# SorF520/D2R

Measured on AMD Instinct MI355X. Metric: samples/sec fwd+bwd, higher is better.
Workload: dtype fp16

## Files before the change

d2r_amd/csrc/attention_impl.inc:

```
typedef H16<E>::v8 E8;
typedef H16<E>::v4 E4;

namespace {

struct MhaArgs {
  const E *q, *k, *v, *res, *dO;
  E *o, *dq, *dk, *dv;
  const float* mask;
  float* lse;
  float* dsum;
  uint32_t drop_thresh;
  float drop_scale;
  uint64_t drop_seed;
  int lkp;
  int64_t ldq, sqb, ldk, skb, ldv, svb, ldo, sob, ldr, srb, ldg, sgb, lddq, sdqb, lddk, sdkb, lddv, sdvb;
  int B, H, Lq, Lk;
  float scale;
};

constexpr int LDW = 72;

template <int DH, int TOTAL, int NTHREADS>
struct RowStage {
  static constexpr int CHUNKS = TOTAL * 8, IT = (CHUNKS + NTHREADS - 1) / NTHREADS;
// ... 9 lines not shown
    }
  }
  __device__ __forceinline__ void store(E* dst, int tid) const {
#pragma unroll
    for (int it = 0; it < IT; ++it) {
      const int c = tid + it * NTHREADS, row = c >> 3, col = (c & 7) * 8;
      if (CHUNKS % NTHREADS == 0 || c < CHUNKS) st_pack<E, 8>(dst + row * LDW + col, v[it]);
    }
  }
};

template <int DH, int TOTAL, int NTHREADS>
__device__ __forceinline__ void fill_rows(E* dst, const E* src, int64_t ld, int valid, int tid) {
  RowStage<DH, TOTAL, NTHREADS> r;
  r.load(src, ld, valid, tid);
  r.store(dst, tid);
}

template <int DH, int TOTAL, int NTHREADS>
__device__ __forceinline__ void fill_rows2(E* d0, const E* s0, int64_t ld0, int v0, E* d1, const E* s1, int64_t ld1, int v1, int tid) {
  RowStage<DH, TOTAL, NTHREADS> r0, r1;
  r0.load(s0, ld0, v0, tid);
  r1.load(s1, ld1, v1, tid);
  r0.store(d0, tid);
  r1.store(d1, tid);
}

__device__ __forceinline__ E8 lds_frag(const E* p) { return *reinterpret_cast<const E8*>(p); }

__device__ __forceinline__ E8 lds_frag_tr(const E* base, int k0, int c0, int tq, int tp) {
  const E* p0 = base + (k0 + tq) * LDW + c0 + tp * 4;
  const E4 lo = H16<E>::tr_read(p0);
  const E4 hi = H16<E>::tr_read(p0 + 16 * LDW);
  return E8{lo[0], lo[1], lo[2], lo[3], hi[0], hi[1], hi[2], hi[3]};
}

__device__ __forceinline__ E8 pack_frag(const f32x4& a, const f32x4& b) {
  return E8{(E)a[0], (E)a[1], (E)a[2], (E)a[3], (E)b[0], (E)b[1], (E)b[2], (E)b[3]};
}

__device__ __forceinline__ float group4_max(float v) {
  v = fmaxf(v, __shfl_xor(v, 16, 64));
  return fmaxf(v, __shfl_xor(v, 32, 64));
}
__device__ __forceinline__ float group4_sum(float v) {
  v += __shfl_xor(v, 16, 64);
  return v + __shfl_xor(v, 32, 64);
}

__device__ __forceinline__ float drop_mult(const MhaArgs& a, uint64_t row_base, int key) {
  return d2r_rand24(a.drop_seed, row_base + (uint64_t)key) >= a.drop_thresh ? a.drop_scale : 0.f;
}

template <int DH, int NK32>
__global__ __launch_bounds__(512) void mha_fwd_kernel(MhaArgs a) {
  constexpr int LKP = NK32 * 32, NKT = NK32 * 2, NDT = DH / 16, NW = 8;
  __shared__ __attribute__((aligned(16))) E Ks[LKP * LDW];
  __shared__ __attribute__((aligned(16))) E Vs[LKP * LDW];
  __shared__ __attribute__((aligned(16))) float Ms[LKP];
  const int tid = threadIdx.x, lane = tid & 63, wave = tid >> 6;
  const int fr = lane & 15, fq = lane >> 4, tq = fr >> 2, tp = fr & 3;
  const int b = blockIdx.x / a.H, h = blockIdx.x % a.H;
  const int nqt = (a.Lq + 15) / 16;
  E8 qn[2];
  auto loadq = [&](int qt) {
    const int qrow = min(qt * 16 + fr, a.Lq - 1);
    const E* Qg = a.q + b * a.sqb + h * DH + (int64_t)qrow * a.ldq;
#pragma unroll
    for (int kk = 0; kk < 2; ++kk) {
      const int col = kk * 32 + fq * 8;
      if (col < DH) {
        qn[kk] = *reinterpret_cast<const E8*>(Qg + col);
      } else {
#pragma unroll
        for (int j = 0; j < 8; ++j) qn[kk][j] = (E)0.f;
      }
    }
  };
  if (wave < nqt) loadq(wave);
  fill_rows2<DH, LKP, 512>(Ks, a.k + b * a.skb + h * DH, a.ldk, a.Lk, Vs, a.v + b * a.svb + h * DH, a.ldv, a.Lk, tid);
  for (int key = tid; key < LKP; key += 512)
    Ms[key] = key < a.Lk ? (a.mask ? a.mask[(int64_t)b * a.Lk + key] : 0.f) : -INFINITY;
  __syncthreads();
  for (int qt = wave; qt < nqt; qt += NW) {
    asm volatile("" ::: "memory");
    const int qrow = qt * 16 + fr;
    const bool qok = qrow < a.Lq;
    E8 qf[2] = {qn[0], qn[1]};
    if (qt + NW < nqt) loadq(qt + NW);
    f32x4 s[NKT];
    float mx = -INFINITY;
#pragma unroll
    for (int t = 0; t < NKT; ++t) {
      f32x4 acc = {0.f, 0.f, 0.f, 0.f};
#pragma unroll
      for (int kk = 0; kk < 2; ++kk)
        acc = H16<E>::mfma32(lds_frag(&Ks[(t * 16 + fr) * LDW + kk * 32 + fq * 8]), qf[kk], acc);
      const f32x4 m4 = *reinterpret_cast<const f32x4*>(&Ms[t * 16 + fq * 4]);
#pragma unroll
      for (int r = 0; r < 4; ++r) {
        acc[r] = acc[r] * a.scale + m4[r];
        mx = fmaxf(mx, acc[r]);
      }
      s[t] = acc;
    }
    mx = group4_max(mx);
    float sum = 0.f;
#pragma unroll
    for (int t = 0; t < NKT; ++t)
#pragma unroll
      for (int r = 0; r < 4; ++r) {
        s[t][r] = __expf(s[t][r] - mx);
        sum += s[t][r];
      }
    sum = group4_sum(sum);
    const float inv = 1.f / sum;
    if (fq == 0 && qok) a.lse[((int64_t)b * a.H + h) * a.Lq + qrow] = mx + logf(sum);
    if (a.drop_thresh) {
      const uint64_t rb = (((uint64_t)b * a.H + h) * a.Lq + (qok ? qrow : 0)) * a.lkp;
#pragma unroll
      for (int t = 0; t < NKT; ++t)
#pragma unroll
        for (int r = 0; r < 4; ++r) s[t][r] *= drop_mult(a, rb, t * 16 + fq * 4 + r);
    }
    f32x4 o[NDT];
#pragma unroll
    for (int dt = 0; dt < NDT; ++dt) o[dt] = f32x4{0.f, 0.f, 0.f, 0.f};
#pragma unroll
    for (int u = 0; u < NK32; ++u) {
      const E8 pf = pack_frag(s[2 * u] * inv, s[2 * u + 1] * inv);
#pragma unroll
      for (int dt = 0; dt < NDT; ++dt)
        o[dt] = H16<E>::mfma32(lds_frag_tr(Vs, u * 32 + fq * 4, dt * 16, tq, tp), pf, o[dt]);
    }
    if (!qok) continue;
    E* Og = a.o + b * a.sob + h * DH + (int64_t)qrow * a.ldo;
    const E* Rg = a.res ? a.res + b * a.srb + h * DH + (int64_t)qrow * a.ldr : nullptr;
#pragma unroll
    for (int dt = 0; dt < NDT; ++dt) {
      const int c = dt * 16 + fq * 4;
      Pack<E, 4> out;
      if (Rg) {
        const Pack<E, 4> rv = ld_pack<E, 4>(Rg + c);
#pragma unroll
        for (int r = 0; r < 4; ++r) out.v[r] = (E)(o[dt][r] + (float)rv.v[r]);
      } else {
#pragma unroll
        for (int r = 0; r < 4; ++r) out.v[r] = (E)o[dt][r];
      }
      st_pack<E, 4>(Og + c, out);
    }
  }
}

template <int DH>
__device__ __forceinline__ E8 global_frag(const E* slice, int64_t ld, int row, int valid, int kk, int fq) {
  const int col = kk * 32 + fq * 8;
  const bool ok = row < valid && col < DH;
  E8 v = *reinterpret_cast<const E8*>(slice + (ok ? (int64_t)row * ld + col : 0));
#pragma unroll
  for (int j = 0; j < 8; ++j) v[j] = ok ? v[j] : (E)0.f;
  return v;
}

template <int DH, int NK32>
__global__ __launch_bounds__(512) void mha_bwd_kernel(MhaArgs a) {
  constexpr int LP = NK32 * 32, NT16 = NK32 * 2, NDT = DH / 16, NW = 8;
  __shared__ __attribute__((aligned(16))) E Xs[LP * LDW];
  __shared__ __attribute__((aligned(16))) E Ys[LP * LDW];
  __shared__ __attribute__((aligned(16))) float Ms[LP];
  __shared__ __attribute__((aligned(16))) float Ls[LP];
  __shared__ __attribute__((aligned(16))) float Ds[LP];
  E* const Ks = Xs;
  E* const Vs = Ys;
  E* const Qs = Xs;
  E* const Gs = Ys;
  const int tid = threadIdx.x, lane = tid & 63, wave = tid >> 6;
  const int fr = lane & 15, fq = lane >> 4, tq = fr >> 2, tp = fr & 3;
  const int b = blockIdx.x / a.H, h = blockIdx.x % a.H;
  const E* Qg = a.q + b * a.sqb + h * DH;
  const E* Kg = a.k + b * a.skb + h * DH;
  const E* Vg = a.v + b * a.svb + h * DH;
  const E* Gg = a.dO + b * a.sgb + h * DH;
  const int nqt = (a.Lq + 15) / 16, nkt = (a.Lk + 15) / 16;
  E8 fx[2], fy[2];
  auto fetch = [&](const E* X, int64_t ldx, const E* Y, int64_t ldy, int row0, int valid) {
#pragma unroll
    for (int kk = 0; kk < 2; ++kk) {
      fx[kk] = global_frag<DH>(X, ldx, row0 + fr, valid, kk, fq);
      fy[kk] = global_frag<DH>(Y, ldy, row0 + fr, valid, kk, fq);
    }
  };
  if (wave < nqt) fetch(Qg, a.ldq, Gg, a.ldg, wave * 16, a.Lq);
  fill_rows2<DH, LP, 512>(Ks, Kg, a.ldk, a.Lk, Vs, Vg, a.ldv, a.Lk, tid);
  for (int i = tid; i < LP; i += 512) {
    Ms[i] = i < a.Lk ? (a.mask ? a.mask[(int64_t)b * a.Lk + i] : 0.f) : -INFINITY;
    Ls[i] = i < a.Lq ? a.lse[((int64_t)b * a.H + h) * a.Lq + i] : INFINITY;
    Ds[i] = 0.f;
  }
  __syncthreads();

  for (int qt = wave; qt < nqt; qt += NW) {
    const int q0 = qt * 16;
    if (qt != wave) fetch(Qg, a.ldq, Gg, a.ldg, q0, a.Lq);
    E8 (&qf)[2] = fx, (&gf)[2] = fy;
    const float lse = Ls[q0 + fr];
    const uint64_t rbA = (((uint64_t)b * a.H + h) * a.Lq + min(q0 + fr, a.Lq - 1)) * a.lkp;
    auto tile = [&](int t, f32x4& pv, f32x4& dpv) {
      f32x4 sa = {0.f, 0.f, 0.f, 0.f}, da = {0.f, 0.f, 0.f, 0.f};
#pragma unroll
      for (int kk = 0; kk < 2; ++kk) {
        sa = H16<E>::mfma32(lds_frag(&Ks[(t * 16 + fr) * LDW + kk * 32 + fq * 8]), qf[kk], sa);
        da = H16<E>::mfma32(lds_frag(&Vs[(t * 16 + fr) * LDW + kk * 32 + fq * 8]), gf[kk], da);
      }
      const f32x4 m4 = *reinterpret_cast<const f32x4*>(&Ms[t * 16 + fq * 4]);
#pragma unroll
      for (int r = 0; r < 4; ++r) sa[r] = __expf(sa[r] * a.scale + m4[r] - lse);
      if (a.drop_thresh) {
#pragma unroll
        for (int r = 0; r < 4; ++r) da[r] *= drop_mult(a, rbA, t * 16 + fq * 4 + r);
      }
      pv = sa;
      dpv = da;
    };
    float dsum = 0.f;
#pragma unroll 2
    for (int t = 0; t < NT16; ++t) {
      f32x4 pv, dpv;
      tile(t, pv, dpv);
#pragma unroll
      for (int r = 0; r < 4; ++r) dsum += pv[r] * dpv[r];
    }
    dsum = group4_sum(dsum);
    if (fq == 0) Ds[q0 + fr] = dsum;
    f32x4 dq[NDT];
#pragma unroll
    for (int dt = 0; dt < NDT; ++dt) dq[dt] = f32x4{0.f, 0.f, 0.f, 0.f};
#pragma unroll 1
    for (int u = 0; u < NK32; ++u) {
      f32x4 p0, p1, d0, d1;
      tile(2 * u, p0, d0);
      tile(2 * u + 1, p1, d1);
#pragma unroll
      for (int r = 0; r < 4; ++r) {
        d0[r] = p0[r] * (d0[r] - dsum) * a.scale;
        d1[r] = p1[r] * (d1[r] - dsum) * a.scale;
      }
      const E8 dsf = pack_frag(d0, d1);
#pragma unroll
      for (int dt = 0; dt < NDT; ++dt)
        dq[dt] = H16<E>::mfma32(lds_frag_tr(Ks, u * 32 + fq * 4, dt * 16, tq, tp), dsf, dq[dt]);
    }
    if (q0 + fr < a.Lq) {
      E* dQg = a.dq + b * a.sdqb + h * DH + (int64_t)(q0 + fr) * a.lddq;
#pragma unroll
      for (int dt = 0; dt < NDT; ++dt) {
        Pack<E, 4> out;
#pragma unroll
        for (int r = 0; r < 4; ++r) out.v[r] = (E)dq[dt][r];
        st_pack<E, 4>(dQg + dt * 16 + fq * 4, out);
      }
    }
  }
  if (wave < nkt) fetch(Kg, a.ldk, Vg, a.ldv, wave * 16, a.Lk);
  __syncthreads();
  fill_rows2<DH, LP, 512>(Qs, Qg, a.ldq, a.Lq, Gs, Gg, a.ldg, a.Lq, tid);
  __syncthreads();

  for (int kt = wave; kt < nkt; kt += NW) {
    const int k0 = kt * 16;
    if (kt != wave) fetch(Kg, a.ldk, Vg, a.ldv, k0, a.Lk);
    E8 (&kf)[2] = fx, (&vf)[2] = fy;
    const float mk = Ms[k0 + fr];
    f32x4 dk[NDT], dv[NDT];
#pragma unroll
    for (int dt = 0; dt < NDT; ++dt) {
      dk[dt] = f32x4{0.f, 0.f, 0.f, 0.f};
      dv[dt] = f32x4{0.f, 0.f, 0.f, 0.f};
    }
#pragma unroll 1
    for (int u = 0; u < NK32; ++u) {
      f32x4 pt[2], dst[2];
#pragma unroll
      for (int half = 0; half < 2; ++half) {
        const int r0 = (u * 2 + half) * 16;
        f32x4 sa = {0.f, 0.f, 0.f, 0.f}, da = {0.f, 0.f, 0.f, 0.f};
#pragma unroll
        for (int kk = 0; kk < 2; ++kk) {
          sa = H16<E>::mfma32(lds_frag(&Qs[(r0 + fr) * LDW + kk * 32 + fq * 8]), kf[kk], sa);
          da = H16<E>::mfma32(lds_frag(&Gs[(r0 + fr) * LDW + kk * 32 + fq * 8]), vf[kk], da);
        }
        const f32x4 l4 = *reinterpret_cast<const f32x4*>(&Ls[r0 + fq * 4]);
        const f32x4 d4 = *reinterpret_cast<const f32x4*>(&Ds[r0 + fq * 4]);
#pragma unroll
        for (int r = 0; r < 4; ++r) {
          const float pv = __expf(sa[r] * a.scale + mk - l4[r]);
          float mlt = 1.f;
          if (a.drop_thresh)
            mlt = drop_mult(a, (((uint64_t)b * a.H + h) * a.Lq + min(r0 + fq * 4 + r, a.Lq - 1)) * a.lkp, min(k0 + fr, a.Lk - 1));
          pt[half][r] = pv * mlt;
          dst[half][r] = pv * (da[r] * mlt - d4[r]) * a.scale;
        }
      }
      const E8 pf = pack_frag(pt[0], pt[1]), dsf = pack_frag(dst[0], dst[1]);
#pragma unroll
      for (int dt = 0; dt < NDT; ++dt) {
        dv[dt] = H16<E>::mfma32(lds_frag_tr(Gs, u * 32 + fq * 4, dt * 16, tq, tp), pf, dv[dt]);
        dk[dt] = H16<E>::mfma32(lds_frag_tr(Qs, u * 32 + fq * 4, dt * 16, tq, tp), dsf, dk[dt]);
      }
    }
    if (k0 + fr < a.Lk) {
      E* dKg = a.dk + b * a.sdkb + h * DH + (int64_t)(k0 + fr) * a.lddk;
      E* dVg = a.dv + b * a.sdvb + h * DH + (int64_t)(k0 + fr) * a.lddv;
#pragma unroll
      for (int dt = 0; dt < NDT; ++dt) {
        Pack<E, 4> ok, ov;
#pragma unroll
        for (int r = 0; r < 4; ++r) {
          ok.v[r] = (E)dk[dt][r];
          ov.v[r] = (E)dv[dt][r];
        }
        st_pack<E, 4>(dKg + dt * 16 + fq * 4, ok);
        st_pack<E, 4>(dVg + dt * 16 + fq * 4, ov);
      }
// ... 247 lines not shown
    for (int u = 0; u < NK32; ++u) {
      f32x4 pt[2], dst[2];
#pragma unroll
      for (int half = 0; half < 2; ++half) {
        const int r0 = (u * 2 + half) * 16;
        f32x4 sa = {0.f, 0.f, 0.f, 0.f}, da = {0.f, 0.f, 0.f, 0.f};
#pragma unroll
        for (int kk = 0; kk < 2; ++kk) {
          sa = H16<E>::mfma32(lds_frag(&Qs[(r0 + fr) * LDW + kk * 32 + fq * 8]), kf[kk], sa);
          da = H16<E>::mfma32(lds_frag(&Gs[(r0 + fr) * LDW + kk * 32 + fq * 8]), vf[kk], da);
        }
        const f32x4 l4 = *reinterpret_cast<const f32x4*>(&Ls[r0 + fq * 4]);
        const f32x4 d4 = *reinterpret_cast<const f32x4*>(&Ds[r0 + fq * 4]);
#pragma unroll
        for (int r = 0; r < 4; ++r) {
          const float pv = __expf(sa[r] * a.scale + mk - l4[r]);
          float mlt = 1.f;
          if (a.drop_thresh)
            mlt = drop_mult(a, (((uint64_t)b * a.H + h) * a.Lq + min(q0 + r0 + fq * 4 + r, a.Lq - 1)) * a.lkp, kok ? krow : 0);
          pt[half][r] = pv * mlt;
          dst[half][r] = pv * (da[r] * mlt - d4[r]) * a.scale;
        }
      }
      const E8 pf = pack_frag(pt[0], pt[1]), dsf = pack_frag(dst[0], dst[1]);
#pragma unroll
      for (int dt = 0; dt < NDT; ++dt) {
        dv[dt] = H16<E>::mfma32(lds_frag_tr(Gs, u * 32 + fq * 4, dt * 16, tq, tp), pf, dv[dt]);
        dk[dt] = H16<E>::mfma32(lds_frag_tr(Qs, u * 32 + fq * 4, dt * 16, tq, tp), dsf, dk[dt]);
      }
    }
  }
  if (!kok) return;
  E* dKg = a.dk + b * a.sdkb + h * DH + (int64_t)krow * a.lddk;
  E* dVg = a.dv + b * a.sdvb + h * DH + (int64_t)krow * a.lddv;
#pragma unroll
  for (int dt = 0; dt < NDT; ++dt) {
    Pack<E, 4> ok, ov;
#pragma unroll
    for (int r = 0; r < 4; ++r) {
      ok.v[r] = (E)dk[dt][r];
      ov.v[r] = (E)dv[dt][r];
    }
    st_pack<E, 4>(dKg + dt * 16 + fq * 4, ok);
    st_pack<E, 4>(dVg + dt * 16 + fq * 4, ov);
  }
}

bool aligned_slice(const void* p, int64_t ld, int64_t sb, int dh) {
  return p && (reinterpret_cast<uintptr_t>(p) & 15u) == 0 && ld % 8 == 0 && sb % 8 == 0 && (dh * 2) % 16 == 0;
}

template <int DH>
void launch_fwd(const MhaArgs& a, int nk32, hipStream_t st) {
  const dim3 grid(a.B * a.H), block(512);
  switch (nk32) {
#define D2R_CASE(N) case N: hipLaunchKernelGGL((mha_fwd_kernel<DH, N>), grid, block, 0, st, a); break;
    D2R_CASE(1) D2R_CASE(2) D2R_CASE(3) D2R_CASE(4) D2R_CASE(5) D2R_CASE(6) D2R_CASE(7) D2R_CASE(8)
#undef D2R_CASE
  }
  d2r_attn_note(D2R_AV_MHA_FWD + DH * 100 + nk32);
}
template <int DH>
void launch_bwd(const MhaArgs& a, int nk32, hipStream_t st) {
  const dim3 grid(a.B * a.H), block(512);
  switch (nk32) {
#define D2R_CASE(N) case N: hipLaunchKernelGGL((mha_bwd_kernel<DH, N>), grid, block, 0, st, a); break;
    D2R_CASE(1) D2R_CASE(2) D2R_CASE(3) D2R_CASE(4) D2R_CASE(5) D2R_CASE(6) D2R_CASE(7) D2R_CASE(8)
#undef D2R_CASE
  }
  d2r_attn_note(D2R_AV_MHA_BWD + DH * 100 + nk32);
}

}

int mha_fwd_run(int dtype, const void* q, int64_t ldq, int64_t sqb, const void* k, int64_t ldk, int64_t skb,
                           const void* v, int64_t ldv, int64_t svb, void* o, int64_t ldo, int64_t sob,
                           const void* residual, int64_t ldr, int64_t srb, const float* mask, float* lse, int B, int H,
                           int Lq, int Lk, int head_dim, float scale, float p_drop, uint64_t seed, void* stream) {
  D2R_REQUIRE(p_drop >= 0.f && p_drop < 1.f, "d2r_mha_fwd: dropout probability must be in [0, 1)");
  D2R_REQUIRE(d2r_mha_supported(dtype, Lq, Lk, head_dim), "d2r_mha_fwd: unsupported (16-bit dtype, head_dim 64|48, L <= 1024 only)");
  D2R_REQUIRE(B >= 1 && H >= 1 && lse, "d2r_mha_fwd: bad arguments");
  D2R_REQUIRE(aligned_slice(q, ldq, sqb, head_dim) && aligned_slice(k, ldk, skb, head_dim) && aligned_slice(v, ldv, svb, head_dim) &&
                  aligned_slice(o, ldo, sob, head_dim) && (!residual || aligned_slice(residual, ldr, srb, head_dim)),
              "d2r_mha_fwd: pointers must be 16-byte aligned, strides multiples of 8 elements");
  MhaArgs a = {};
  a.q = (const E*)q, a.k = (const E*)k, a.v = (const E*)v, a.res = (const E*)residual, a.o = (E*)o;
  a.mask = mask, a.lse = lse;
  a.ldq = ldq, a.sqb = sqb, a.ldk = ldk, a.skb = skb, a.ldv = ldv, a.svb = svb, a.ldo = ldo, a.sob = sob, a.ldr = ldr, a.srb = srb;
  a.B = B, a.H = H, a.Lq = Lq, a.Lk = Lk, a.scale = scale;
  a.drop_thresh = p_drop > 0.f ? d2r_drop_threshold(p_drop) : 0u, a.drop_scale = 1.f / (1.f - p_drop), a.drop_seed = seed, a.lkp = (Lk + 7) / 8 * 8;
  if (Lq > 256 || Lk > 256) {
    const dim3 grid(d2r_cdiv(Lq, LB), B * H);
    if (head_dim == 64) hipLaunchKernelGGL(mha_long_fwd_kernel<64>, grid, dim3(512), 0, (hipStream_t)stream, a);
    else hipLaunchKernelGGL(mha_long_fwd_kernel<48>, grid, dim3(512), 0, (hipStream_t)stream, a);
    d2r_attn_note(D2R_AV_MHA_LONG_FWD + head_dim * 100);
    return d2r_check_launch("d2r_mha_fwd(long)");
  }
  const int nk32 = d2r_cdiv(Lk, 32);
  if (head_dim == 64) launch_fwd<64>(a, nk32, (hipStream_t)stream);
  else launch_fwd<48>(a, nk32, (hipStream_t)stream);
  return d2r_check_launch("d2r_mha_fwd");
}

int mha_bwd_run(int dtype, const void* q, int64_t ldq, int64_t sqb, const void* k, int64_t ldk, int64_t skb,
                           const void* v, int64_t ldv, int64_t svb, const void* dO, int64_t ldg, int64_t sgb,
                           const float* mask, const float* lse, float* dsum, void* dq, int64_t lddq, int64_t sdqb, void* dk,
                           int64_t lddk, int64_t sdkb, void* dv, int64_t lddv, int64_t sdvb, int B, int H, int Lq, int Lk,
                           int head_dim, float scale, float p_drop, uint64_t seed, void* stream) {
  D2R_REQUIRE(p_drop >= 0.f && p_drop < 1.f, "d2r_mha_bwd: dropout probability must be in [0, 1)");
  D2R_REQUIRE(d2r_mha_supported(dtype, Lq, Lk, head_dim), "d2r_mha_bwd: unsupported (16-bit dtype, head_dim 64|48, L <= 1024 only)");
  D2R_REQUIRE((Lq <= 256 && Lk <= 256) || dsum, "d2r_mha_bwd: sequences above 256 tokens need the dsum scratch ([B, H, Lq] fp32)");
  D2R_REQUIRE(B >= 1 && H >= 1 && lse, "d2r_mha_bwd: bad arguments");
  D2R_REQUIRE(aligned_slice(q, ldq, sqb, head_dim) && aligned_slice(k, ldk, skb, head_dim) && aligned_slice(v, ldv, svb, head_dim) &&
                  aligned_slice(dO, ldg, sgb, head_dim) && aligned_slice(dq, lddq, sdqb, head_dim) &&
                  aligned_slice(dk, lddk, sdkb, head_dim) && aligned_slice(dv, lddv, sdvb, head_dim),
              "d2r_mha_bwd: pointers must be 16-byte aligned, strides multiples of 8 elements");
  MhaArgs a = {};
// ... 307 lines not shown
```

d2r_amd/csrc/rowops.hip:

```cpp
#include "common.h"

template <typename TX, typename TY, int MAXPL>
__global__ __launch_bounds__(256) void softmax_fwd_kernel(const TX* __restrict__ X, TY* __restrict__ Y, int64_t ld,
                                                          int64_t rows, int cols, float scale,
                                                          const float* __restrict__ mask, int64_t rows_per_mask) {
  const int lane = threadIdx.x & 63;
  const int64_t row = (int64_t)blockIdx.x * 4 + (threadIdx.x >> 6);
  if (row >= rows) return;
  const TX* x = X + row * ld;
  const float* mk = mask ? mask + (row / rows_per_mask) * cols : nullptr;
  float v[MAXPL];
  float mx = -INFINITY;
#pragma unroll
  for (int i = 0; i < MAXPL; ++i) {
    const int c = lane + i * 64;
    if (c < cols) {
      float t = scale * to_f<TX>(x[c]);
      if (mk) t += mk[c];
      v[i] = t;
      mx = fmaxf(mx, t);
    } else {
      v[i] = -INFINITY;
    }
  }
// ... 206 lines not shown
#pragma unroll
  for (int i = 0; i < MAXP; ++i) {
    const int pk = lane + i * 64, pc = pk < npk ? pk : 0;
    px[i] = ld_pack<T, VEC>(x + pc * VEC);
#pragma unroll
    for (int j = 0; j < VEC; j += 4) {
      const float4 g4 = *reinterpret_cast<const float4*>(gamma + pc * VEC + j);
      const float4 b4 = *reinterpret_cast<const float4*>(beta + pc * VEC + j);
      gm[i][j] = g4.x, gm[i][j + 1] = g4.y, gm[i][j + 2] = g4.z, gm[i][j + 3] = g4.w;
      bt[i][j] = b4.x, bt[i][j + 1] = b4.y, bt[i][j + 2] = b4.z, bt[i][j + 3] = b4.w;
    }
  }
  __builtin_amdgcn_sched_barrier(0);
#pragma unroll
  for (int i = 0; i < MAXP; ++i) {
    const float mk = lane + i * 64 < npk ? 1.f : 0.f;
#pragma unroll
    for (int j = 0; j < VEC; ++j) {
      v[i][j] = to_f<T>(px[i].v[j]);
      s += v[i][j] * mk;
    }
  }
  const float mu = wave_sum(s) / D;
  float q = 0.f;
#pragma unroll
  for (int i = 0; i < MAXP; ++i) {
    const int pk = lane + i * 64;
    if (pk < npk) {
#pragma unroll
      for (int j = 0; j < VEC; ++j) {
        const float d = v[i][j] - mu;
        q += d * d;
      }
    }
  }
  const float rs = rsqrtf(wave_sum(q) / D + eps);
  if (lane == 0) {
    mean[row] = mu;
    rstd[row] = rs;
  }
  T* y = Y + row * D;
#pragma unroll
  for (int i = 0; i < MAXP; ++i) {
    const int pk = lane + i * 64;
    if (pk < npk) {
      Pack<T, VEC> o;
#pragma unroll
      for (int j = 0; j < VEC; ++j) o.v[j] = from_f<T>((v[i][j] - mu) * rs * gm[i][j] + bt[i][j]);
      st_pack<T, VEC>(y + pk * VEC, o);
    }
  }
}

template <typename T, int MAXP>
__global__ __launch_bounds__(256) void layernorm_bwd_kernel(const T* __restrict__ dY, const T* __restrict__ X,
                                                            const float* __restrict__ gamma,
                                                            const float* __restrict__ mean,
                                                            const float* __restrict__ rstd, int64_t rows, int D,
                                                            T* __restrict__ dX, float* __restrict__ ws,
                                                            const T* __restrict__ dres) {
  constexpr int VEC = PackOf<T>::N;
  extern __shared__ __attribute__((aligned(16))) float sh[];
  const int lane = threadIdx.x & 63, wave = threadIdx.x >> 6;
  const int npk = D / VEC;
  float dg[MAXP][VEC], db[MAXP][VEC], gm[MAXP][VEC];
#pragma unroll
  for (int i = 0; i < MAXP; ++i) {
    const int pk = lane + i * 64;
#pragma unroll
    for (int j = 0; j < VEC; ++j) {
      dg[i][j] = 0.f;
      db[i][j] = 0.f;
      gm[i][j] = (pk < npk) ? gamma[pk * VEC + j] : 0.f;
    }
  }
  struct RowRegs {
    Pack<T, VEC> x[MAXP], dy[MAXP], r[MAXP];
    float mu, rs;
  };
  auto fetch = [&](int64_t row, RowRegs& q) {
    q.mu = mean[row];
    q.rs = rstd[row];
#pragma unroll
    for (int i = 0; i < MAXP; ++i) {
      const int pk = lane + i * 64;
      if (pk < npk) {
        q.x[i] = ld_pack<T, VEC>(X + row * D + pk * VEC);
        q.dy[i] = ld_pack<T, VEC>(dY + row * D + pk * VEC);
        if (dres) q.r[i] = ld_pack<T, VEC>(dres + row * D + pk * VEC);
      }
    }
  };
  const int64_t step = (int64_t)gridDim.x * 4;
  int64_t row = (int64_t)blockIdx.x * 4 + wave;
  RowRegs cur, nxt;
  if (row < rows) fetch(row, cur);
  for (; row < rows; row += step) {
    const bool more = row + step < rows;
    if (more) fetch(row + step, nxt);
    const float mu = cur.mu, rs = cur.rs;
    float xh[MAXP][VEC], g[MAXP][VEC];
    float s1 = 0.f, s2 = 0.f;
#pragma unroll
    for (int i = 0; i < MAXP; ++i) {
      const int pk = lane + i * 64;
      if (pk < npk) {
#pragma unroll
        for (int j = 0; j < VEC; ++j) {
          const float d = to_f<T>(cur.dy[i].v[j]);
          xh[i][j] = (to_f<T>(cur.x[i].v[j]) - mu) * rs;
          g[i][j] = d * gm[i][j];
          s1 += g[i][j];
          s2 += g[i][j] * xh[i][j];
          dg[i][j] += d * xh[i][j];
          db[i][j] += d;
        }
      }
    }
    s1 = wave_sum(s1) / D;
    s2 = wave_sum(s2) / D;
    T* dx = dX + row * D;
#pragma unroll
    for (int i = 0; i < MAXP; ++i) {
      const int pk = lane + i * 64;
      if (pk < npk) {
        Pack<T, VEC> o;
        if (dres) {
#pragma unroll
          for (int j = 0; j < VEC; ++j) o.v[j] = from_f<T>(rs * (g[i][j] - s1 - xh[i][j] * s2) + to_f<T>(cur.r[i].v[j]));
        } else {
#pragma unroll
          for (int j = 0; j < VEC; ++j) o.v[j] = from_f<T>(rs * (g[i][j] - s1 - xh[i][j] * s2));
        }
        st_pack<T, VEC>(dx + pk * VEC, o);
      }
    }
    if (more) cur = nxt;
  }
#pragma unroll
  for (int i = 0; i < MAXP; ++i) {
    const int pk = lane + i * 64;
    if (pk < npk) {
#pragma unroll
      for (int j = 0; j < VEC; j += 4) {
        Pack<float, 4> pg, pb;
#pragma unroll
        for (int u = 0; u < 4; ++u) pg.v[u] = dg[i][j + u], pb.v[u] = db[i][j + u];
        st_pack<float, 4>(&sh[(wave * 2 + 0) * D + pk * VEC + j], pg);
        st_pack<float, 4>(&sh[(wave * 2 + 1) * D + pk * VEC + j], pb);
      }
    }
  }
  __syncthreads();
  for (int c = threadIdx.x; c < 2 * D; c += 256) {
    const float t = sh[0 * 2 * D + c] + sh[1 * 2 * D + c] + sh[2 * 2 * D + c] + sh[3 * 2 * D + c];
    ws[(int64_t)blockIdx.x * 2 * D + c] = t;
  }
}

static int ln_blocks(int64_t rows) {
  int64_t b = (rows + 3) / 4;
  return (int)(b < 1 ? 1 : (b > 512 ? 512 : b));
}

extern "C" size_t d2r_layernorm_bwd_workspace(int64_t rows, int D) {
  return (size_t)ln_blocks(rows) * 2 * D * sizeof(float);
}

template <typename T>
static int ln_check(const char* fn, int D) {
  constexpr int VEC = PackOf<T>::N;
  if (D % VEC != 0 || D < VEC || D > 64 * VEC * 4) return d2r_fail(D2R_ERR_INVALID, "%s: D=%d unsupported (need D %% %d == 0 and D <= %d)", fn, D, VEC, 64 * VEC * 4);
  return D2R_OK;
}

extern "C" int d2r_layernorm_fwd(int dtype, const void* X, const float* gamma, const float* beta, float eps,
                                 int64_t rows, int D, void* Y, float* mean, float* rstd, void* stream) {
  D2R_REQUIRE(X && Y && gamma && beta && mean && rstd, "d2r_layernorm_fwd: null pointer");
  D2R_REQUIRE(d2r_aligned16(X) && d2r_aligned16(Y), "d2r_layernorm_fwd: X/Y must be 16-byte aligned");
  if (rows == 0) return D2R_OK;
  hipStream_t st = (hipStream_t)stream;
  dim3 grid(d2r_cdiv(rows, 4)), block(256);
  if (dtype == D2R_BF16) {
    if (int rc = ln_check<bf16_t>("d2r_layernorm_fwd", D)) return rc;
    if (D <= 64 * 8 * 2) hipLaunchKernelGGL((layernorm_fwd_kernel<bf16_t, 2>), grid, block, 0, st, (const bf16_t*)X, gamma, beta, eps, rows, D, (bf16_t*)Y, mean, rstd);
    else hipLaunchKernelGGL((layernorm_fwd_kernel<bf16_t, 4>), grid, block, 0, st, (const bf16_t*)X, gamma, beta, eps, rows, D, (bf16_t*)Y, mean, rstd);
  } else if (dtype == D2R_F16) {
    if (int rc = ln_check<f16_t>("d2r_layernorm_fwd", D)) return rc;
    if (D <= 64 * 8 * 2) hipLaunchKernelGGL((layernorm_fwd_kernel<f16_t, 2>), grid, block, 0, st, (const f16_t*)X, gamma, beta, eps, rows, D, (f16_t*)Y, mean, rstd);
    else hipLaunchKernelGGL((layernorm_fwd_kernel<f16_t, 4>), grid, block, 0, st, (const f16_t*)X, gamma, beta, eps, rows, D, (f16_t*)Y, mean, rstd);
  } else if (dtype == D2R_F32) {
    if (int rc = ln_check<float>("d2r_layernorm_fwd", D)) return rc;
    hipLaunchKernelGGL((layernorm_fwd_kernel<float, 4>), grid, block, 0, st, (const float*)X, gamma, beta, eps, rows, D, (float*)Y, mean, rstd);
  } else {
    return d2r_fail(D2R_ERR_INVALID, "d2r_layernorm_fwd: bad dtype %d", dtype);
  }
  return d2r_check_launch("d2r_layernorm_fwd");
}

extern "C" int d2r_layernorm_bwd_ex(int dtype, const void* dY, const void* X, const float* gamma, const float* mean,
                                    const float* rstd, int64_t rows, int D, void* dX, const void* dres, float* dgamma,
                                    float* dbeta, int accumulate, void* workspace, size_t workspace_bytes, void* stream) {
  D2R_REQUIRE(dY && X && gamma && mean && rstd && dX && ((dgamma != nullptr) == (dbeta != nullptr)), "d2r_layernorm_bwd: null pointer");
  D2R_REQUIRE(d2r_aligned16(X) && d2r_aligned16(dY) && d2r_aligned16(dX) && d2r_aligned16(dres), "d2r_layernorm_bwd: tensors must be 16-byte aligned");
  if (workspace_bytes < d2r_layernorm_bwd_workspace(rows, D) || !workspace)
    return d2r_fail(D2R_ERR_WORKSPACE, "d2r_layernorm_bwd: workspace %zu < %zu", workspace_bytes, d2r_layernorm_bwd_workspace(rows, D));
  hipStream_t st = (hipStream_t)stream;
  const int nb = ln_blocks(rows);
  float* ws = (float*)workspace;
  const size_t shmem = (size_t)4 * 2 * D * sizeof(float);
  if (dtype == D2R_BF16) {
    if (int rc = ln_check<bf16_t>("d2r_layernorm_bwd", D)) return rc;
    if (D <= 64 * 8 * 2) hipLaunchKernelGGL((layernorm_bwd_kernel<bf16_t, 2>), dim3(nb), dim3(256), shmem, st, (const bf16_t*)dY, (const bf16_t*)X, gamma, mean, rstd, rows, D, (bf16_t*)dX, ws, (const bf16_t*)dres);
    else hipLaunchKernelGGL((layernorm_bwd_kernel<bf16_t, 4>), dim3(nb), dim3(256), shmem, st, (const bf16_t*)dY, (const bf16_t*)X, gamma, mean, rstd, rows, D, (bf16_t*)dX, ws, (const bf16_t*)dres);
  } else if (dtype == D2R_F16) {
    if (int rc = ln_check<f16_t>("d2r_layernorm_bwd", D)) return rc;
    if (D <= 64 * 8 * 2) hipLaunchKernelGGL((layernorm_bwd_kernel<f16_t, 2>), dim3(nb), dim3(256), shmem, st, (const f16_t*)dY, (const f16_t*)X, gamma, mean, rstd, rows, D, (f16_t*)dX, ws, (const f16_t*)dres);
    else hipLaunchKernelGGL((layernorm_bwd_kernel<f16_t, 4>), dim3(nb), dim3(256), shmem, st, (const f16_t*)dY, (const f16_t*)X, gamma, mean, rstd, rows, D, (f16_t*)dX, ws, (const f16_t*)dres);
  } else if (dtype == D2R_F32) {
    if (int rc = ln_check<float>("d2r_layernorm_bwd", D)) return rc;
    if (D <= 64 * 4 * 3) hipLaunchKernelGGL((layernorm_bwd_kernel<float, 3>), dim3(nb), dim3(256), shmem, st, (const float*)dY, (const float*)X, gamma, mean, rstd, rows, D, (float*)dX, ws, (const float*)dres);
    else hipLaunchKernelGGL((layernorm_bwd_kernel<float, 4>), dim3(nb), dim3(256), shmem, st, (const float*)dY, (const float*)X, gamma, mean, rstd, rows, D, (float*)dX, ws, (const float*)dres);
  } else {
    return d2r_fail(D2R_ERR_INVALID, "d2r_layernorm_bwd: bad dtype %d", dtype);
  }
  if (int rc = d2r_check_launch("d2r_layernorm_bwd")) return rc;
  if (!dgamma) return D2R_OK;
  hipLaunchKernelGGL(ln_sum_partials_kernel, dim3(d2r_cdiv(2 * D, 16)), dim3(256), 0, st, ws, nb, D, dgamma, dbeta, accumulate);
  return d2r_check_launch("d2r_layernorm_bwd(sum)");
}

extern "C" int d2r_layernorm_bwd_sum_grouped(const void* const* partials, float* const* dgamma, float* const* dbeta, int n, int64_t rows,
                                             int D, int accumulate, void* stream) {
  D2R_REQUIRE(partials && dgamma && dbeta && n >= 0 && rows >= 1 && D >= 1, "d2r_layernorm_bwd_sum_grouped: bad argument");
  const int nb = ln_blocks(rows);
  for (int i0 = 0; i0 < n; i0 += 32) {
    const int m = n - i0 < 32 ? n - i0 : 32;
    LnSumGroup grp;
    for (int i = 0; i < m; ++i) {
      D2R_REQUIRE(partials[i0 + i] && dgamma[i0 + i] && dbeta[i0 + i], "d2r_layernorm_bwd_sum_grouped: null pointer in problem %d", i0 + i);
      grp.ws[i] = (const float*)partials[i0 + i], grp.dg[i] = dgamma[i0 + i], grp.db[i] = dbeta[i0 + i];
    }
    hipLaunchKernelGGL(ln_sum_partials_grouped_kernel, dim3(d2r_cdiv(2 * D, 16), m), dim3(256), 0, (hipStream_t)stream, grp, nb, D, accumulate);
    if (int rc = d2r_check_launch("d2r_layernorm_bwd_sum_grouped")) return rc;
  }
  return D2R_OK;
}

extern "C" int d2r_layernorm_bwd(int dtype, const void* dY, const void* X, const float* gamma, const float* mean,
                                 const float* rstd, int64_t rows, int D, void* dX, float* dgamma, float* dbeta,
                                 void* workspace, size_t workspace_bytes, void* stream) {
  return d2r_layernorm_bwd_ex(dtype, dY, X, gamma, mean, rstd, rows, D, dX, nullptr, dgamma, dbeta, 0, workspace,
                              workspace_bytes, stream);
}

template <typename T, int MAXP>
__global__ __launch_bounds__(256) void l2norm_fwd_kernel(const T* __restrict__ X, T* __restrict__ Y,
                                                         float* __restrict__ norm, int64_t rows, int D) {
  constexpr int VEC = PackOf<T>::N;
  const int lane = threadIdx.x & 63;
  const int64_t row = (int64_t)blockIdx.x * 4 + (threadIdx.x >> 6);
  if (row >= rows) return;
  const int npk = D / VEC;
  const T* x = X + row * D;
  float v[MAXP][VEC];
  float q = 0.f;
#pragma unroll
  for (int i = 0; i < MAXP; ++i) {
    const int pk = lane + i * 64;
    if (pk < npk) {
      Pack<T, VEC> p = ld_pack<T, VEC>(x + pk * VEC);
#pragma unroll
      for (int j = 0; j < VEC; ++j) {
        v[i][j] = to_f<T>(p.v[j]);
        q += v[i][j] * v[i][j];
// ... 192 lines not shown
```

Before: 1544.

## Split attention heads across two blocks and rework layernorm backward row scheduling

The forward and backward attention kernels now launch two blocks per (batch, head) along grid.y. Each block handles half the query tiles, and each wave handles exactly one tile, replacing the strided multi-tile loop. For short sequences, smaller 4-wave blocks are used with occupancy hints. The backward pass now computes dsum for the other half's query tiles redundantly and can prefetch two fragment sets at once. Separately, layernorm backward switches from grid-stride rows to contiguous rows-per-wave chunks sized to fill the GPU. It recomputes xh and g in the store phase instead of keeping them in registers, using asm barriers to cut register pressure. The trade is more parallelism against duplicated K/V loads, repeated dsum work and added redundant arithmetic, and the one-tile-per-wave mapping assumes the query tiles fit within a block.

```diff
diff --git a/d2r_amd/csrc/attention_impl.inc b/d2r_amd/csrc/attention_impl.inc
--- a/d2r_amd/csrc/attention_impl.inc
+++ b/d2r_amd/csrc/attention_impl.inc
@@ -85,9 +85,13 @@
   return d2r_rand24(a.drop_seed, row_base + (uint64_t)key) >= a.drop_thresh ? a.drop_scale : 0.f;
 }
 
-template <int DH, int NK32>
-__global__ __launch_bounds__(512) void mha_fwd_kernel(MhaArgs a) {
-  constexpr int LKP = NK32 * 32, NKT = NK32 * 2, NDT = DH / 16, NW = 8;
+constexpr int MHA_SPLIT = 2;
+__device__ __forceinline__ int mha_part_lo(int n, int p) { return p * ((n + 1) / 2); }
+__device__ __forceinline__ int mha_part_hi(int n, int p) { return p ? n : (n + 1) / 2; }
+
+template <int DH, int NK32, int NW>
+__global__ __launch_bounds__(NW * 64, NW == 8 ? 4 : 3) void mha_fwd_kernel(MhaArgs a) {
+  constexpr int LKP = NK32 * 32, NKT = NK32 * 2, NDT = DH / 16;
   __shared__ __attribute__((aligned(16))) E Ks[LKP * LDW];
   __shared__ __attribute__((aligned(16))) E Vs[LKP * LDW];
   __shared__ __attribute__((aligned(16))) float Ms[LKP];
@@ -95,6 +99,9 @@
   const int fr = lane & 15, fq = lane >> 4, tq = fr >> 2, tp = fr & 3;
   const int b = blockIdx.x / a.H, h = blockIdx.x % a.H;
   const int nqt = (a.Lq + 15) / 16;
+  const int qt = mha_part_lo(nqt, blockIdx.y) + wave;
+  const bool mine = qt < mha_part_hi(nqt, blockIdx.y);
+  if (mha_part_lo(nqt, blockIdx.y) >= nqt) return;
   E8 qn[2];
   auto loadq = [&](int qt) {
     const int qrow = min(qt * 16 + fr, a.Lq - 1);
@@ -110,17 +117,15 @@
       }
     }
   };
-  if (wave < nqt) loadq(wave);
-  fill_rows2<DH, LKP, 512>(Ks, a.k + b * a.skb + h * DH, a.ldk, a.Lk, Vs, a.v + b * a.svb + h * DH, a.ldv, a.Lk, tid);
-  for (int key = tid; key < LKP; key += 512)
+  if (mine) loadq(qt);
+  fill_rows2<DH, LKP, NW * 64>(Ks, a.k + b * a.skb + h * DH, a.ldk, a.Lk, Vs, a.v + b * a.svb + h * DH, a.ldv, a.Lk, tid);
+  for (int key = tid; key < LKP; key += NW * 64)
     Ms[key] = key < a.Lk ? (a.mask ? a.mask[(int64_t)b * a.Lk + key] : 0.f) : -INFINITY;
   __syncthreads();
-  for (int qt = wave; qt < nqt; qt += NW) {
-    asm volatile("" ::: "memory");
+  if (mine) {
     const int qrow = qt * 16 + fr;
     const bool qok = qrow < a.Lq;
     E8 qf[2] = {qn[0], qn[1]};
-    if (qt + NW < nqt) loadq(qt + NW);
     f32x4 s[NKT];
     float mx = -INFINITY;
 #pragma unroll
@@ -166,7 +171,7 @@
       for (int dt = 0; dt < NDT; ++dt)
         o[dt] = H16<E>::mfma32(lds_frag_tr(Vs, u * 32 + fq * 4, dt * 16, tq, tp), pf, o[dt]);
     }
-    if (!qok) continue;
+    if (!qok) return;
     E* Og = a.o + b * a.sob + h * DH + (int64_t)qrow * a.ldo;
     const E* Rg = a.res ? a.res + b * a.srb + h * DH + (int64_t)qrow * a.ldr : nullptr;
 #pragma unroll
@@ -197,8 +202,8 @@
 }
 
 template <int DH, int NK32>
-__global__ __launch_bounds__(512) void mha_bwd_kernel(MhaArgs a) {
-  constexpr int LP = NK32 * 32, NT16 = NK32 * 2, NDT = DH / 16, NW = 8;
+__global__ __launch_bounds__(NK32 <= 4 ? 256 : 512) void mha_bwd_kernel(MhaArgs a) {
+  constexpr int LP = NK32 * 32, NT16 = NK32 * 2, NDT = DH / 16, NW = NK32 <= 4 ? 4 : 8, NT = NW * 64;
   __shared__ __attribute__((aligned(16))) E Xs[LP * LDW];
   __shared__ __attribute__((aligned(16))) E Ys[LP * LDW];
   __shared__ __attribute__((aligned(16))) float Ms[LP];
@@ -216,26 +221,45 @@
   const E* Vg = a.v + b * a.svb + h * DH;
   const E* Gg = a.dO + b * a.sgb + h * DH;
   const int nqt = (a.Lq + 15) / 16, nkt = (a.Lk + 15) / 16;
-  E8 fx[2], fy[2];
-  auto fetch = [&](const E* X, int64_t ldx, const E* Y, int64_t ldy, int row0, int valid) {
+  const int part = blockIdx.y;
+  if (mha_part_lo(nqt, part) >= nqt && mha_part_lo(nkt, part) >= nkt) return;
+  const int qt_own = mha_part_lo(nqt, part) + wave, qt_oth = mha_part_lo(nqt, part ^ 1) + wave;
+  const bool own_ok = qt_own < mha_part_hi(nqt, part);
+  const bool oth_ok = qt_oth < mha_part_hi(nqt, part ^ 1) && mha_part_lo(nkt, part) < nkt;
+  const int kt = mha_part_lo(nkt, part) + wave;
+  const bool key_ok = kt < mha_part_hi(nkt, part);
+  constexpr bool TWO_BUF = NW == 4;
+  E8 fx[2], fy[2], gx[2], gy[2];
+  auto fetch = [&](E8 (&x)[2], E8 (&y)[2], const E* X, int64_t ldx, const E* Y, int64_t ldy, int row0, int valid) {
 #pragma unroll
     for (int kk = 0; kk < 2; ++kk) {
-      fx[kk] = global_frag<DH>(X, ldx, row0 + fr, valid, kk, fq);
-      fy[kk] = global_frag<DH>(Y, ldy, row0 + fr, valid, kk, fq);
+      x[kk] = global_frag<DH>(X, ldx, row0 + fr, valid, kk, fq);
+      y[kk] = global_frag<DH>(Y, ldy, row0 + fr, valid, kk, fq);
     }
   };
-  if (wave < nqt) fetch(Qg, a.ldq, Gg, a.ldg, wave * 16, a.Lq);
-  fill_rows2<DH, LP, 512>(Ks, Kg, a.ldk, a.Lk, Vs, Vg, a.ldv, a.Lk, tid);
-  for (int i = tid; i < LP; i += 512) {
+  if (oth_ok) fetch(fx, fy, Qg, a.ldq, Gg, a.ldg, qt_oth * 16, a.Lq);
+  else if (own_ok) fetch(fx, fy, Qg, a.ldq, Gg, a.ldg, qt_own * 16, a.Lq);
+  if (TWO_BUF && oth_ok && own_ok) fetch(gx, gy, Qg, a.ldq, Gg, a.ldg, qt_own * 16, a.Lq);
+  fill_rows2<DH, LP, NT>(Ks, Kg, a.ldk, a.Lk, Vs, Vg, a.ldv, a.Lk, tid);
+  for (int i = tid; i < LP; i += NT) {
     Ms[i] = i < a.Lk ? (a.mask ? a.mask[(int64_t)b * a.Lk + i] : 0.f) : -INFINITY;
     Ls[i] = i < a.Lq ? a.lse[((int64_t)b * a.H + h) * a.Lq + i] : INFINITY;
     Ds[i] = 0.f;
   }
   __syncthreads();
 
-  for (int qt = wave; qt < nqt; qt += NW) {
-    const int q0 = qt * 16;
-    if (qt != wave) fetch(Qg, a.ldq, Gg, a.ldg, q0, a.Lq);
+#pragma unroll 1
+  for (int pass = 0; pass < 2; ++pass) {
+    if (!(pass ? own_ok : oth_ok)) continue;
+    const int q0 = (pass ? qt_own : qt_oth) * 16;
+    if (pass && oth_ok) {
+      if (TWO_BUF) {
+#pragma unroll
+        for (int kk = 0; kk < 2; ++kk) fx[kk] = gx[kk], fy[kk] = gy[kk];
+      } else {
+        fetch(fx, fy, Qg, a.ldq, Gg, a.ldg, q0, a.Lq);
+      }
+    }
     E8 (&qf)[2] = fx, (&gf)[2] = fy;
     const float lse = Ls[q0 + fr];
     const uint64_t rbA = (((uint64_t)b * a.H + h) * a.Lq + min(q0 + fr, a.Lq - 1)) * a.lkp;
@@ -266,6 +290,7 @@
     }
     dsum = group4_sum(dsum);
     if (fq == 0) Ds[q0 + fr] = dsum;
+    if (!pass) continue;
     f32x4 dq[NDT];
 #pragma unroll
     for (int dt = 0; dt < NDT; ++dt) dq[dt] = f32x4{0.f, 0.f, 0.f, 0.f};
@@ -295,14 +320,14 @@
       }
     }
   }
-  if (wave < nkt) fetch(Kg, a.ldk, Vg, a.ldv, wave * 16, a.Lk);
+  if (mha_part_lo(nkt, part) >= nkt) return;
+  if (key_ok) fetch(fx, fy, Kg, a.ldk, Vg, a.ldv, kt * 16, a.Lk);
   __syncthreads();
-  fill_rows2<DH, LP, 512>(Qs, Qg, a.ldq, a.Lq, Gs, Gg, a.ldg, a.Lq, tid);
+  fill_rows2<DH, LP, NT>(Qs, Qg, a.ldq, a.Lq, Gs, Gg, a.ldg, a.Lq, tid);
   __syncthreads();
 
-  for (int kt = wave; kt < nkt; kt += NW) {
+  if (key_ok) {
     const int k0 = kt * 16;
-    if (kt != wave) fetch(Kg, a.ldk, Vg, a.ldv, k0, a.Lk);
     E8 (&kf)[2] = fx, (&vf)[2] = fy;
     const float mk = Ms[k0 + fr];
     f32x4 dk[NDT], dv[NDT];
@@ -656,9 +681,14 @@
 
 template <int DH>
 void launch_fwd(const MhaArgs& a, int nk32, hipStream_t st) {
-  const dim3 grid(a.B * a.H), block(512);
+  const dim3 grid(a.B * a.H, MHA_SPLIT);
+  const bool w4 = a.Lq <= 128;
   switch (nk32) {
-#define D2R_CASE(N) case N: hipLaunchKernelGGL((mha_fwd_kernel<DH, N>), grid, block, 0, st, a); break;
+#define D2R_CASE(N)                                                                            \
+  case N:                                                                                      \
+    if (w4) hipLaunchKernelGGL((mha_fwd_kernel<DH, N, 4>), grid, dim3(256), 0, st, a);         \
+    else hipLaunchKernelGGL((mha_fwd_kernel<DH, N, 8>), grid, dim3(512), 0, st, a);            \
+    break;
     D2R_CASE(1) D2R_CASE(2) D2R_CASE(3) D2R_CASE(4) D2R_CASE(5) D2R_CASE(6) D2R_CASE(7) D2R_CASE(8)
 #undef D2R_CASE
   }
@@ -666,7 +696,7 @@
 }
 template <int DH>
 void launch_bwd(const MhaArgs& a, int nk32, hipStream_t st) {
-  const dim3 grid(a.B * a.H), block(512);
+  const dim3 grid(a.B * a.H, MHA_SPLIT), block(nk32 <= 4 ? 256 : 512);
   switch (nk32) {
 #define D2R_CASE(N) case N: hipLaunchKernelGGL((mha_bwd_kernel<DH, N>), grid, block, 0, st, a); break;
     D2R_CASE(1) D2R_CASE(2) D2R_CASE(3) D2R_CASE(4) D2R_CASE(5) D2R_CASE(6) D2R_CASE(7) D2R_CASE(8)
diff --git a/d2r_amd/csrc/rowops.hip b/d2r_amd/csrc/rowops.hip
--- a/d2r_amd/csrc/rowops.hip
+++ b/d2r_amd/csrc/rowops.hip
@@ -282,11 +282,22 @@
   }
 }
 
+template <typename P>
+__device__ __forceinline__ void ln_opaque(P& p) {
+  static_assert(sizeof(P) % 4 == 0, "whole registers");
+  uint32_t w[sizeof(P) / 4];
+  __builtin_memcpy(w, &p, sizeof(P));
+#pragma unroll
+  for (unsigned k = 0; k < sizeof(P) / 4; ++k) asm volatile("" : "+v"(w[k]));
+  __builtin_memcpy(&p, w, sizeof(P));
+}
+
+constexpr int LN_BWD_WAVES = 4, LN_BWD_OCC = 3;
 template <typename T, int MAXP>
-__global__ __launch_bounds__(256) void layernorm_bwd_kernel(const T* __restrict__ dY, const T* __restrict__ X,
+__global__ __launch_bounds__(LN_BWD_WAVES * 64, MAXP <= 2 ? LN_BWD_OCC : 1) void layernorm_bwd_kernel(const T* __restrict__ dY, const T* __restrict__ X,
                                                             const float* __restrict__ gamma,
                                                             const float* __restrict__ mean,
-                                                            const float* __restrict__ rstd, int64_t rows, int D,
+                                                            const float* __restrict__ rstd, int64_t rows, int rpw, int D,
                                                             T* __restrict__ dX, float* __restrict__ ws,
                                                             const T* __restrict__ dres) {
   constexpr int VEC = PackOf<T>::N;
@@ -294,16 +305,6 @@
   const int lane = threadIdx.x & 63, wave = threadIdx.x >> 6;
   const int npk = D / VEC;
   float dg[MAXP][VEC], db[MAXP][VEC], gm[MAXP][VEC];
-#pragma unroll
-  for (int i = 0; i < MAXP; ++i) {
-    const int pk = lane + i * 64;
-#pragma unroll
-    for (int j = 0; j < VEC; ++j) {
-      dg[i][j] = 0.f;
-      db[i][j] = 0.f;
-      gm[i][j] = (pk < npk) ? gamma[pk * VEC + j] : 0.f;
-    }
-  }
   struct RowRegs {
     Pack<T, VEC> x[MAXP], dy[MAXP], r[MAXP];
     float mu, rs;
@@ -321,15 +322,25 @@
       }
     }
   };
-  const int64_t step = (int64_t)gridDim.x * 4;
-  int64_t row = (int64_t)blockIdx.x * 4 + wave;
+  int64_t row = ((int64_t)blockIdx.x * LN_BWD_WAVES + wave) * rpw;
+  const int64_t row_end = row + rpw < rows ? row + rpw : rows;
   RowRegs cur, nxt;
-  if (row < rows) fetch(row, cur);
-  for (; row < rows; row += step) {
-    const bool more = row + step < rows;
-    if (more) fetch(row + step, nxt);
-    const float mu = cur.mu, rs = cur.rs;
-    float xh[MAXP][VEC], g[MAXP][VEC];
+  if (row < row_end) fetch(row, cur);
+  if (row + 1 < row_end) fetch(row + 1, nxt);
+#pragma unroll
+  for (int i = 0; i < MAXP; ++i) {
+    const int pk = lane + i * 64;
+#pragma unroll
+    for (int j = 0; j < VEC; ++j) {
+      dg[i][j] = 0.f;
+      db[i][j] = 0.f;
+      gm[i][j] = (pk < npk) ? gamma[pk * VEC + j] : 0.f;
+    }
+  }
+  for (int64_t first = row; row < row_end; ++row) {
+    const bool more = row + 1 < row_end;
+    if (more && row != first) fetch(row + 1, nxt);
+    float mu = cur.mu, rs = cur.rs;
     float s1 = 0.f, s2 = 0.f;
 #pragma unroll
     for (int i = 0; i < MAXP; ++i) {
@@ -338,29 +349,32 @@
 #pragma unroll
         for (int j = 0; j < VEC; ++j) {
           const float d = to_f<T>(cur.dy[i].v[j]);
-          xh[i][j] = (to_f<T>(cur.x[i].v[j]) - mu) * rs;
-          g[i][j] = d * gm[i][j];
-          s1 += g[i][j];
-          s2 += g[i][j] * xh[i][j];
-          dg[i][j] += d * xh[i][j];
+          const float xh = (to_f<T>(cur.x[i].v[j]) - mu) * rs;
+          const float g = d * gm[i][j];
+          s1 += g;
+          s2 += g * xh;
+          dg[i][j] += d * xh;
           db[i][j] += d;
         }
       }
     }
     s1 = wave_sum(s1) / D;
     s2 = wave_sum(s2) / D;
+    ln_opaque(mu), ln_opaque(rs);
+#pragma unroll
+    for (int i = 0; i < MAXP; ++i) ln_opaque(cur.x[i]), ln_opaque(cur.dy[i]);
     T* dx = dX + row * D;
 #pragma unroll
     for (int i = 0; i < MAXP; ++i) {
       const int pk = lane + i * 64;
       if (pk < npk) {
         Pack<T, VEC> o;
-        if (dres) {
-#pragma unroll
-          for (int j = 0; j < VEC; ++j) o.v[j] = from_f<T>(rs * (g[i][j] - s1 - xh[i][j] * s2) + to_f<T>(cur.r[i].v[j]));
-        } else {
-#pragma unroll
-          for (int j = 0; j < VEC; ++j) o.v[j] = from_f<T>(rs * (g[i][j] - s1 - xh[i][j] * s2));
+#pragma unroll
+        for (int j = 0; j < VEC; ++j) {
+          const float xh = (to_f<T>(cur.x[i].v[j]) - mu) * rs;
+          const float g = to_f<T>(cur.dy[i].v[j]) * gm[i][j];
+          const float v = rs * (g - s1 - xh * s2);
+          o.v[j] = from_f<T>(dres ? v + to_f<T>(cur.r[i].v[j]) : v);
         }
         st_pack<T, VEC>(dx + pk * VEC, o);
       }
@@ -382,15 +396,19 @@
     }
   }
   __syncthreads();
-  for (int c = threadIdx.x; c < 2 * D; c += 256) {
+  for (int c = threadIdx.x; c < 2 * D; c += LN_BWD_WAVES * 64) {
     const float t = sh[0 * 2 * D + c] + sh[1 * 2 * D + c] + sh[2 * 2 * D + c] + sh[3 * 2 * D + c];
     ws[(int64_t)blockIdx.x * 2 * D + c] = t;
   }
 }
 
+static int ln_rows_per_wave(int64_t rows) {
+  const int64_t cap = 256 * 4 * LN_BWD_OCC, r = (rows + cap - 1) / cap;
+  return (int)(r < 1 ? 1 : r);
+}
 static int ln_blocks(int64_t rows) {
-  int64_t b = (rows + 3) / 4;
-  return (int)(b < 1 ? 1 : (b > 512 ? 512 : b));
+  const int64_t rpw = ln_rows_per_wave(rows), waves = (rows + rpw - 1) / rpw, b = (waves + LN_BWD_WAVES - 1) / LN_BWD_WAVES;
+  return (int)(b < 1 ? 1 : b);
 }
 
 extern "C" size_t d2r_layernorm_bwd_workspace(int64_t rows, int D) {
@@ -436,21 +454,21 @@
   if (workspace_bytes < d2r_layernorm_bwd_workspace(rows, D) || !workspace)
     return d2r_fail(D2R_ERR_WORKSPACE, "d2r_layernorm_bwd: workspace %zu < %zu", workspace_bytes, d2r_layernorm_bwd_workspace(rows, D));
   hipStream_t st = (hipStream_t)stream;
-  const int nb = ln_blocks(rows);
+  const int nb = ln_blocks(rows), rpw = ln_rows_per_wave(rows);
   float* ws = (float*)workspace;
   const size_t shmem = (size_t)4 * 2 * D * sizeof(float);
   if (dtype == D2R_BF16) {
     if (int rc = ln_check<bf16_t>("d2r_layernorm_bwd", D)) return rc;
-    if (D <= 64 * 8 * 2) hipLaunchKernelGGL((layernorm_bwd_kernel<bf16_t, 2>), dim3(nb), dim3(256), shmem, st, (const bf16_t*)dY, (const bf16_t*)X, gamma, mean, rstd, rows, D, (bf16_t*)dX, ws, (const bf16_t*)dres);
-    else hipLaunchKernelGGL((layernorm_bwd_kernel<bf16_t, 4>), dim3(nb), dim3(256), shmem, st, (const bf16_t*)dY, (const bf16_t*)X, gamma, mean, rstd, rows, D, (bf16_t*)dX, ws, (const bf16_t*)dres);
+    if (D <= 64 * 8 * 2) hipLaunchKernelGGL((layernorm_bwd_kernel<bf16_t, 2>), dim3(nb), dim3(LN_BWD_WAVES * 64), shmem, st, (const bf16_t*)dY, (const bf16_t*)X, gamma, mean, rstd, rows, rpw, D, (bf16_t*)dX, ws, (const bf16_t*)dres);
+    else hipLaunchKernelGGL((layernorm_bwd_kernel<bf16_t, 4>), dim3(nb), dim3(LN_BWD_WAVES * 64), shmem, st, (const bf16_t*)dY, (const bf16_t*)X, gamma, mean, rstd, rows, rpw, D, (bf16_t*)dX, ws, (const bf16_t*)dres);
   } else if (dtype == D2R_F16) {
     if (int rc = ln_check<f16_t>("d2r_layernorm_bwd", D)) return rc;
-    if (D <= 64 * 8 * 2) hipLaunchKernelGGL((layernorm_bwd_kernel<f16_t, 2>), dim3(nb), dim3(256), shmem, st, (const f16_t*)dY, (const f16_t*)X, gamma, mean, rstd, rows, D, (f16_t*)dX, ws, (const f16_t*)dres);
-    else hipLaunchKernelGGL((layernorm_bwd_kernel<f16_t, 4>), dim3(nb), dim3(256), shmem, st, (const f16_t*)dY, (const f16_t*)X, gamma, mean, rstd, rows, D, (f16_t*)dX, ws, (const f16_t*)dres);
+    if (D <= 64 * 8 * 2) hipLaunchKernelGGL((layernorm_bwd_kernel<f16_t, 2>), dim3(nb), dim3(LN_BWD_WAVES * 64), shmem, st, (const f16_t*)dY, (const f16_t*)X, gamma, mean, rstd, rows, rpw, D, (f16_t*)dX, ws, (const f16_t*)dres);
+    else hipLaunchKernelGGL((layernorm_bwd_kernel<f16_t, 4>), dim3(nb), dim3(LN_BWD_WAVES * 64), shmem, st, (const f16_t*)dY, (const f16_t*)X, gamma, mean, rstd, rows, rpw, D, (f16_t*)dX, ws, (const f16_t*)dres);
   } else if (dtype == D2R_F32) {
     if (int rc = ln_check<float>("d2r_layernorm_bwd", D)) return rc;
-    if (D <= 64 * 4 * 3) hipLaunchKernelGGL((layernorm_bwd_kernel<float, 3>), dim3(nb), dim3(256), shmem, st, (const float*)dY, (const float*)X, gamma, mean, rstd, rows, D, (float*)dX, ws, (const float*)dres);
-    else hipLaunchKernelGGL((layernorm_bwd_kernel<float, 4>), dim3(nb), dim3(256), shmem, st, (const float*)dY, (const float*)X, gamma, mean, rstd, rows, D, (float*)dX, ws, (const float*)dres);
+    if (D <= 64 * 4 * 3) hipLaunchKernelGGL((layernorm_bwd_kernel<float, 3>), dim3(nb), dim3(LN_BWD_WAVES * 64), shmem, st, (const float*)dY, (const float*)X, gamma, mean, rstd, rows, rpw, D, (float*)dX, ws, (const float*)dres);
+    else hipLaunchKernelGGL((layernorm_bwd_kernel<float, 4>), dim3(nb), dim3(LN_BWD_WAVES * 64), shmem, st, (const float*)dY, (const float*)X, gamma, mean, rstd, rows, rpw, D, (float*)dX, ws, (const float*)dres);
   } else {
     return d2r_fail(D2R_ERR_INVALID, "d2r_layernorm_bwd: bad dtype %d", dtype);
   }
```

New measurement: 1536. Within noise of the previous version (-0.5%).
